# felixzhu17/Reranking-Multimodal-Retrievers

Hardware: AMD Instinct MI355X
Metric: reranked query x candidate pairs/sec at K=100, seq_len=512 (higher is better)
Workload: dtype fp16

## Files before the change

reranking-multimodal-retrievers_amd/build.py:

```python
from __future__ import annotations

import os
import subprocess
import sys
from concurrent.futures import ThreadPoolExecutor

HERE = os.path.dirname(os.path.abspath(__file__))
CSRC = os.path.join(HERE, "csrc")
LIB = os.path.join(HERE, "librerank_mi355.so")
SOURCES = ["rr_api.hip", "gemm_bf16.hip", "gemm_fp8.hip", "attention_bf16.hip", "elementwise.hip", "head.hip", "pair_assembly.hip", "li_scores.hip", "passage_bank.hip",
           "pair_tokenizer.cpp"]
HEADERS = [os.path.join(CSRC, "rr_common.h"), os.path.join(os.path.dirname(HERE), "include", "rerank_mi355.h"),
           os.path.join(os.path.dirname(HERE), "include", "rerank_mi355_diag.h"),
           os.path.join(CSRC, "unicode_tables.h")]
HIPCC = os.environ.get("HIPCC", "/opt/rocm/bin/hipcc")
FLAGS = ["--offload-arch=gfx950", "-O3", "-fPIC", "-std=c++17", "-Wall", "-Wno-unused-function", "-fno-slp-vectorize",
         *os.environ.get("RR_HIPCC_EXTRA", "").split()]
EXTRA = {"attention_bf16.hip": ["-fno-honor-nans", "-mno-amdgpu-ieee"]}


def _stale(target: str, deps) -> bool:
    if not os.path.exists(target):
        return True
    t = os.path.getmtime(target)
    return any(os.path.getmtime(d) > t for d in deps)


OBJDUMP = os.path.join(os.path.dirname(os.path.dirname(HIPCC)), "lib", "llvm", "bin", "llvm-objdump")
NO_PACKED_F32 = ["gemm_bf16.o", "gemm_fp8.o", "elementwise.o", "pair_assembly.o", "li_scores.o", "passage_bank.o"]


def check_no_packed_f32(obj: str) -> None:
    import re
    import shutil
    import tempfile
    if not os.path.exists(OBJDUMP):
        raise RuntimeError(f"{OBJDUMP} not found: cannot verify the packed-f32 rule for {obj}")
    d = tempfile.mkdtemp(prefix="rr_isa_")
    try:
        local = os.path.join(d, os.path.basename(obj))
        shutil.copy(obj, local)
        subprocess.run([OBJDUMP, "--offloading", local], cwd=d, capture_output=True, text=True, check=True)
        dev = [f for f in os.listdir(d) if "gfx950" in f]
        if len(dev) != 1:
            raise RuntimeError(f"no gfx950 code object in {obj}")
        dis = subprocess.run([OBJDUMP, "-d", os.path.join(d, dev[0])], capture_output=True, text=True, check=True).stdout
        bad = re.findall(r"v_pk_(?:add|mul)_f32[^\n]*", dis)
        ins = [l.split("//")[0].strip() for l in dis.splitlines() if l.startswith("\t")]
        for i, l in enumerate(ins):
            if i and l.startswith("v_pk_fma_f32") and ins[i - 1].startswith("s_waitcnt"):
                bad.append(l + "   (behind " + ins[i - 1] + ")")
        if bad:
            raise RuntimeError(f"{os.path.basename(obj)}: {len(bad)} packed-f32 instructions in the device code (first: {bad[0].strip()}); "
                               "build with -fno-slp-vectorize (reranking-multimodal-retrievers_amd/build.py FLAGS)")
    finally:
        shutil.rmtree(d, ignore_errors=True)


LAST_BUILD: dict = {}


def build_library(force: bool = False, verbose: bool = False) -> str:
    import json
    import time
    lib_existed = os.path.exists(LIB)
    objdir = os.path.join(HERE, "build")
    os.makedirs(objdir, exist_ok=True)
    jobs = []
    for s in SOURCES:
        src = os.path.join(CSRC, s)
        obj = os.path.join(objdir, os.path.splitext(s)[0] + ".o")
        if force or _stale(obj, [src] + HEADERS):
            if s.endswith(".cpp"):
                jobs.append([HIPCC, "-O2", "-fPIC", "-std=c++17", "-Wall", "-pthread", "-c", src, "-o", obj])
            else:
                jobs.append([HIPCC, *FLAGS, *EXTRA.get(s, []), "-c", src, "-o", obj])

    def run(cmd):
        if verbose:
            print(" ".join(cmd), flush=True)
        r = subprocess.run(cmd, capture_output=True, text=True)
        if r.returncode != 0:
            raise RuntimeError("hipcc failed:\n" + " ".join(cmd) + "\n" + r.stdout + r.stderr)
        return r.stderr

    with ThreadPoolExecutor(max_workers=4) as ex:
        list(ex.map(run, jobs))
    objs = [os.path.join(objdir, os.path.splitext(s)[0] + ".o") for s in SOURCES]
    if force or jobs or _stale(LIB, objs):
        for o in NO_PACKED_F32:
            obj = os.path.join(objdir, o)
            try:
                check_no_packed_f32(obj)
            except RuntimeError:
                os.remove(obj)
                raise
        run([HIPCC, "--offload-arch=gfx950", "-shared", "-fPIC", "-pthread", "-o", LIB, *objs])
        linked = True
    else:
        linked = False
    LAST_BUILD.clear()
    LAST_BUILD.update(compiled=[os.path.basename(j[-3]) for j in jobs], linked=linked, reused_prebuilt_library=lib_existed and not linked,
                      forced=bool(force), when=time.strftime("%Y-%m-%dT%H:%M:%S"))
    try:
        with open(os.path.join(objdir, "build_record.json"), "w") as f:
            json.dump(LAST_BUILD, f, indent=1)
    except OSError:
        pass
    return LIB


if __name__ == "__main__":
    print(build_library(force="--force" in sys.argv, verbose=True))
```

reranking-multimodal-retrievers_amd/csrc/gemm_bf16.hip:

```cpp
#include "rr_common.h"

#include <atomic>
#include <cstdlib>
#include <mutex>

#ifndef RR_EPI_DIAG
#define RR_EPI_DIAG 0
#endif

namespace {

constexpr int BK = 64;
__device__ __forceinline__ int k_walk_reversed(int n0) { return (n0 >> 10) & 1; }

__device__ __forceinline__ void lds_barrier() {
  asm volatile("s_waitcnt lgkmcnt(0)" ::: "memory");
  __builtin_amdgcn_s_barrier();
  asm volatile("" ::: "memory");
}

template <int N>
__device__ __forceinline__ void wait_vmcnt() {
  if constexpr (N == 0) asm volatile("s_waitcnt vmcnt(0)" ::: "memory");
  else if constexpr (N == 2) asm volatile("s_waitcnt vmcnt(2)" ::: "memory");
  else if constexpr (N == 4) asm volatile("s_waitcnt vmcnt(4)" ::: "memory");
  else if constexpr (N == 6) asm volatile("s_waitcnt vmcnt(6)" ::: "memory");
  else if constexpr (N == 8) asm volatile("s_waitcnt vmcnt(8)" ::: "memory");
  else if constexpr (N == 10) asm volatile("s_waitcnt vmcnt(10)" ::: "memory");
  else if constexpr (N == 12) asm volatile("s_waitcnt vmcnt(12)" ::: "memory");
  else if constexpr (N == 16) asm volatile("s_waitcnt vmcnt(16)" ::: "memory");
  else if constexpr (N == 24) asm volatile("s_waitcnt vmcnt(24)" ::: "memory");
  else static_assert(N < 0, "add the vmcnt literal");
}

template <int PIECES, int MAXT>
__device__ __forceinline__ void wait_tiles(int tiles_in_flight) {
  if constexpr (MAXT >= 2) { if (tiles_in_flight >= 2) { wait_vmcnt<2 * PIECES>(); return; } }
  if constexpr (MAXT >= 1) { if (tiles_in_flight >= 1) { wait_vmcnt<PIECES>(); return; } }
  wait_vmcnt<0>();
}

__device__ __forceinline__ float fast_erf(float x) {
  const float ax = fabsf(x);
  const float t = __builtin_amdgcn_rcpf(fmaf(0.3275911f, ax, 1.0f));
  float p = fmaf(1.061405429f, t, -1.453152027f);
  p = fmaf(p, t, 1.421413741f);
  p = fmaf(p, t, -0.284496736f);
  p = fmaf(p, t, 0.254829592f);
  const float e = __expf(-ax * ax);
  const float r = fmaf(-p * t, e, 1.0f);
  return copysignf(r, x);
}
__device__ __forceinline__ float tanh_fast(float x) { return 1.0f - 2.0f * __builtin_amdgcn_rcpf(__expf(2.0f * x) + 1.0f); }
__device__ __forceinline__ float qgelu_fast(float x) { return x * __builtin_amdgcn_rcpf(1.0f + __expf(-1.702f * x)); }
__device__ __forceinline__ float gelu_fast(float x) { return gelu_erf_fast(x); }

struct LnResid {
  const float2* stats;
  const float* gamma;
  const float* beta;
  bf16_t* x16;
  int ldx;
  float2* part;
  int nparts;
  const float2* in_stats;
  const float* csum;
  int flags;
  const bf16_t* r_hi;
  const bf16_t* r_lo;
  int ld16;
  bf16_t* lo_out;
};
__device__ __forceinline__ float dpp_f(float old, float v, int ctrl, int row_mask, bool bound) {
  return __builtin_bit_cast(float, ctrl == 0x111 ? __builtin_amdgcn_update_dpp(__builtin_bit_cast(int, old), __builtin_bit_cast(int, v), 0x111, 0xf, 0xf, true)
                                   : ctrl == 0x112 ? __builtin_amdgcn_update_dpp(__builtin_bit_cast(int, old), __builtin_bit_cast(int, v), 0x112, 0xf, 0xf, true)
                                   : ctrl == 0x114 ? __builtin_amdgcn_update_dpp(__builtin_bit_cast(int, old), __builtin_bit_cast(int, v), 0x114, 0xf, 0xf, true)
                                   : ctrl == 0x118 ? __builtin_amdgcn_update_dpp(__builtin_bit_cast(int, old), __builtin_bit_cast(int, v), 0x118, 0xf, 0xf, true)
                                                   : __builtin_amdgcn_update_dpp(__builtin_bit_cast(int, old), __builtin_bit_cast(int, v), 0x142, 0xa, 0xf, false));
}
__device__ __forceinline__ float group32_sum(float v) {
  v += dpp_f(0.f, v, 0x111, 0xf, true);
  v += dpp_f(0.f, v, 0x112, 0xf, true);
  v += dpp_f(0.f, v, 0x114, 0xf, true);
  v += dpp_f(0.f, v, 0x118, 0xf, true);
  v += dpp_f(0.f, v, 0x142, 0xa, false);
  const int vi = __builtin_bit_cast(int, v);
  const float lo = __builtin_bit_cast(float, __builtin_amdgcn_readlane(vi, 31));
  const float hi = __builtin_bit_cast(float, __builtin_amdgcn_readlane(vi, 63));
  return (threadIdx.x & 32) ? hi : lo;
}
// ... 537 lines not shown
            const int gm = row_base + r, gcol = n0 + c * (16 / ES);
            const bool ok = i < ROWS * CPR && gm < M && gcol < N;
            float4 x = ok ? *(const float4*)(resid + (size_t)gm * ldr + gcol) : make_float4(0.f, 0.f, 0.f, 0.f);
            if (ln.stats) {
              const int gm_s = __builtin_amdgcn_readfirstlane(min(gm, M - 1));
              const float2 st2 = ln.stats[gm_s];
              x = make_float4((x.x - st2.x) * st2.y * lg.x + lb.x, (x.y - st2.x) * st2.y * lg.y + lb.y,
                              (x.z - st2.x) * st2.y * lg.z + lb.z, (x.w - st2.x) * st2.y * lg.w + lb.w);
            }
            rv[u] = x;
          }
        }
        static_assert((ROWS * CPR) % (512 * UNR) == 0, "every thread runs every step (cross-lane sums below)");
#pragma unroll
        for (int u = 0; u < UNR; ++u) {
          const int i = i0 + u * 512, r = i / CPR, c = i - r * CPR;
          const int gm = row_base + r, gcol = n0 + c * (16 / ES);
          const bool ok = i < ROWS * CPR && gm < M && gcol < N;
          float4 f = make_float4(0.f, 0.f, 0.f, 0.f);
          if (ok) {
            uint4 v = *(const uint4*)(lds + r * PITCH + c * 16);
            if (EPI == EPI_BIAS_RESID_F32) {
              f = __builtin_bit_cast(float4, v);
              f.x += rv[u].x; f.y += rv[u].y; f.z += rv[u].z; f.w += rv[u].w;
              v = __builtin_bit_cast(uint4, f);
            }
            *(uint4*)((char*)Cv + ((size_t)gm * ldc + gcol) * ES) = v;
          }
          if (EPI == EPI_BIAS_RESID_F32) { if (ln.x16) fold_emit<DT>(ln, f, ok, gm, gcol, N); }
        }
      }
      if (pass + 1 < NPASS) lds_barrier();
    }
  } else {
#pragma unroll
    for (int q = 0; q < 4; ++q) {
      const int hA = q >> 1, hB = q & 1;
#pragma unroll
      for (int nt = 0; nt < 2; ++nt) {
        const int gn = n0 + hB * 128 + wc * 32 + nt * 16 + (lane >> 4) * 4;
        if (gn >= N) continue;
        const float4 bv = (bias && !bias_done) ? *(const float4*)(bias + gn) : make_float4(0.f, 0.f, 0.f, 0.f);
#pragma unroll
        for (int mt = 0; mt < 4; ++mt) {
          const int gm = m0 + hA * 128 + wr * 64 + mt * 16 + (lane & 15);
          if (gm >= M) continue;
          float v0 = acc[q][nt][mt][0] + bv.x, v1 = acc[q][nt][mt][1] + bv.y, v2 = acc[q][nt][mt][2] + bv.z,
                v3 = acc[q][nt][mt][3] + bv.w;
          if (EPI == EPI_BIAS_GELU_BF16) { v0 = gelu_fast(v0); v1 = gelu_fast(v1); v2 = gelu_fast(v2); v3 = gelu_fast(v3); }
          if (EPI == EPI_BIAS_TANH_BF16) { v0 = tanh_fast(v0); v1 = tanh_fast(v1); v2 = tanh_fast(v2); v3 = tanh_fast(v3); }
          if (EPI == EPI_BIAS_QGELU_BF16) { v0 = qgelu_fast(v0); v1 = qgelu_fast(v1); v2 = qgelu_fast(v2); v3 = qgelu_fast(v3); }
          if (EPI == EPI_BIAS_RESID_F32) {
            const float4 rv = ln_apply(*(const float4*)(resid + (size_t)gm * ldr + gn), ln, gm, gn);
            v0 += rv.x; v1 += rv.y; v2 += rv.z; v3 += rv.w;
          }
          if (F32_OUT) *(float4*)((float*)Cv + (size_t)gm * ldc + gn) = make_float4(v0, v1, v2, v3);
          else *(uint2*)((bf16_t*)Cv + (size_t)gm * ldc + gn) = make_uint2(pack2<DT>(v0, v1), pack2<DT>(v2, v3));
        }
      }
    }
  }
  stamp(stamps, 3);
}

template <int EPI, int DT, int SPLIT = 0, int DIAG = 0, bool FOLD = false>
__global__ __launch_bounds__(512) void gemm_kernel_hp(const bf16_t* __restrict__ A, int lda,
                                                     const bf16_t* __restrict__ W, int ldw,
                                                     const float* __restrict__ bias,
                                                     const float* __restrict__ resid, int ldr,
                                                     void* __restrict__ Cv, int ldc, int M, int N, int Kd,
                                                     int tiles_n, int nwg, unsigned long long* stamps, LnResid ln,
                                                     int stagger_unit) {
  const bool mrev = stagger_unit >= 1000;
  if (mrev) stagger_unit -= 1000;
  const int GROUP = stagger_unit >= 50 && stagger_unit <= 55 ? (2 << (stagger_unit - 50))
                    : (stagger_unit == 56 || Kd > 1024 || (tiles_n <= 4 && stagger_unit != 57)) ? 1 : 8;
  if (stagger_unit >= 100) {
    const int n = (int)(blockIdx.x & 7) * (stagger_unit - 100);
    for (int i = 0; i < n; ++i) __builtin_amdgcn_s_sleep(4);
  }
  stamp(stamps, 0);
  constexpr int BM = 256, BN = 256, HALF = 128 * 128;
  constexpr bool FOLD_IN = FOLD && EPI != EPI_BIAS_RESID_F32, FOLD_OUT = FOLD && EPI == EPI_BIAS_RESID_F32;
  extern __shared__ __attribute__((aligned(16))) char lds[];

  const int bid = blockIdx.x, gstep = (int)(gridDim.x >> 3);
  const int xcd = bid & 7, q8 = nwg >> 3, r8 = nwg & 7;
  const int chunk0 = xcd < r8 ? xcd * (q8 + 1) : r8 * (q8 + 1) + (xcd - r8) * q8, chunk_n = q8 + (xcd < r8 ? 1 : 0);
  int li = bid >> 3;
  if (li >= chunk_n) return;
  int m0, n0;
  const int tiles_m = nwg / tiles_n;
  const bool serp = stagger_unit != 59;
  int krev = 0;
  auto tile_origin = [&](int gidx, int& m0_, int& n0_) {
    const int per_group = GROUP * tiles_n, grp = gidx / per_group, r = gidx - grp * per_group;
    const int rows = min(GROUP, tiles_m - grp * GROUP);
    const int tn = r / rows, tm = grp * GROUP + (r - tn * rows);
    m0_ = tm * BM;
    n0_ = tn * BN;
    krev = serp ? k_walk_reversed(n0_) : 0;
  };
  tile_origin(chunk0 + (mrev ? chunk_n - 1 - li : li), m0, n0);

  const int tid = threadIdx.x, lane = tid & 63;
  const int wave = __builtin_amdgcn_readfirstlane(tid >> 6);
  const int wr = wave >> 2, wc = wave & 3;

  uint32_t so_a0[2], so_a1[2], so_b0[2], so_b1[2];
  const bf16_t *a_tile, *w_tile;
#define RR_SETUP_SRC(m0_, n0_)                                                                          \
  _Pragma("unroll") for (int i = 0; i < 2; ++i) {                                                       \
    const int r = (wave * 2 + i) * 8 + (lane >> 3);                       \
    const int c = (lane & 7) ^ ((r >> 1) & 7);                                                          \
    so_a0[i] = (uint32_t)(((size_t)min(r, M - 1 - (m0_)) * lda + c * 8) * 2);                           \
    so_a1[i] = (uint32_t)(((size_t)min(128 + r, M - 1 - (m0_)) * lda + c * 8) * 2);                     \
    so_b0[i] = (uint32_t)(((size_t)min(r, N - 1 - (n0_)) * ldw + c * 8) * 2);                           \
    so_b1[i] = (uint32_t)(((size_t)min(128 + r, N - 1 - (n0_)) * ldw + c * 8) * 2);                     \
  }                                                                                                     \
  a_tile = A + (size_t)(m0_) * lda;                                                                     \
  w_tile = W + (size_t)(n0_) * ldw;
  RR_SETUP_SRC(m0, n0)
  const uint32_t lds_base = lds_addr(lds);
  const int nk = Kd / BK, H = 4 * nk;
#define RR_DMA(t_, J)                                                                                             \
  {                                                                                                               \
    const uint32_t dst_ = __builtin_amdgcn_readfirstlane(lds_base + (((t_) & 1) * 4 + (J)) * HALF + wave * 2048); \
    const int tk_ = krev ? nk - 1 - (t_) : (t_);                      \
    const void* sb_ = ((J) == 0 || (J) == 3) ? (const void*)(a_tile + (size_t)tk_ * BK) : (const void*)(w_tile + (size_t)tk_ * BK); \
    const uint32_t* so_ = (J) == 0 ? so_a0 : (J) == 3 ? so_a1 : (J) == 1 ? so_b0 : so_b1;                         \
    glds16_so(sb_, so_[0], dst_);                                                                                 \
    glds16_so(sb_, so_[1], dst_ + 1024);                                                                          \
  }
  auto wait_half = [&](int h_need, int h_last) {
    if (h_need >= H) return;
    const int after = h_last - h_need;
    if (after >= 3) wait_vmcnt<6>();
    else if (after == 2) wait_vmcnt<4>();
    else if (after == 1) wait_vmcnt<2>();
    else wait_vmcnt<0>();
  };

  const int a_off = swz128(wr * 64 + (lane & 15), lane >> 4);
  const int b_off = swz128(wc * 32 + (lane & 15), lane >> 4);
  const int lds_dup = (DIAG == 3 && (stagger_unit == 62 || stagger_unit == 63)) ? stagger_unit - 61 : 0;
  auto dup_read = [&](const char* p_) {
    if constexpr (DIAG == 3) {
      for (int d_ = 0; d_ < lds_dup; ++d_) {
        f32x4 scratch_;
        asm volatile("ds_read_b128 %0, %1" : "=v"(scratch_) : "v"(lds_addr(p_)) : "memory");
      }
    }
  };
  auto read_a = [&](const char* slot, int ks, bf16x8 (&f)[4]) {
    const char* b = slot + (ks ? (a_off ^ 64) : a_off);
#pragma unroll
    for (int mt = 0; mt < 4; ++mt) { f[mt] = *(const bf16x8*)(b + mt * 2048); dup_read(b + mt * 2048); }
  };
  auto read_b = [&](const char* slot, int ks, bf16x8 (&f)[2]) {
    const char* b = slot + (ks ? (b_off ^ 64) : b_off);
#pragma unroll
    for (int nt = 0; nt < 2; ++nt) { f[nt] = *(const bf16x8*)(b + nt * 2048); dup_read(b + nt * 2048); }
  };

  f32x4 acc[4][2][4];

  bf16x8 AF0[4], AF1[4], B0K0[2], B0K1[2], B1K0[2], B1K1[2];

#define RR_BLK(Q, AF, BF)                                                                          \
  _Pragma("unroll") for (int nt = 0; nt < 2; ++nt) _Pragma("unroll") for (int mt = 0; mt < 4; ++mt)  \
      acc[Q][nt][mt] = mfma16<DT>(BF[nt], AF[mt], acc[Q][nt][mt]);
#define RR_SBAR() __builtin_amdgcn_sched_barrier(0)
#define RR_PRIO(p) __builtin_amdgcn_s_setprio(p);

  constexpr int PARAM_OFF = 152 * 1024;
  auto stage_params = [&](int m0_, int n0_) {
    int lane_ = lane;
    asm volatile("" : "+v"(lane_));
    const int lane = lane_;
    if constexpr (FOLD_IN) {
      const int d = wave * 64 + lane;
      glds4_so(ln.in_stats + m0_, (uint32_t)((min(d >> 1, M - 1 - m0_) * 2 + (d & 1)) * 4),
               __builtin_amdgcn_readfirstlane(lds_base + PARAM_OFF + wave * 256));
    }
    if (wave < 4) {
      if (bias) glds4_so(bias + n0_, (uint32_t)(min(wave * 64 + lane, N - 1 - n0_) * 4),
                         __builtin_amdgcn_readfirstlane(lds_base + PARAM_OFF + 2048 + wave * 256));
    } else if (FOLD_IN) {
      glds4_so(ln.csum + n0_, (uint32_t)(min((wave - 4) * 64 + lane, N - 1 - n0_) * 4),
               __builtin_amdgcn_readfirstlane(lds_base + PARAM_OFF + 3072 + (wave - 4) * 256));
    }
    if (EPI == EPI_BIAS_RESID_F32 && ln.stats) {
      const int d = wave * 64 + lane;
      glds4_so(ln.stats + m0_, (uint32_t)((min(d >> 1, M - 1 - m0_) * 2 + (d & 1)) * 4),
               __builtin_amdgcn_readfirstlane(lds_base + PARAM_OFF + 6144 + wave * 256));
      glds4_so((wave < 4 ? ln.gamma : ln.beta) + n0_, (uint32_t)(min((wave & 3) * 64 + lane, N - 1 - n0_) * 4),
               __builtin_amdgcn_readfirstlane(lds_base + PARAM_OFF + 4096 + (wave >> 2) * 1024 + (wave & 3) * 256));
    }
  };
  if (!bias) {
    if (tid < 256) *(float*)(lds + PARAM_OFF + 2048 + tid * 4) = 0.f;
// ... 64 lines not shown
    if (d1) RR_DMA(t + 1, 3)                                  \
    RR_SBAR();                                                                                             \
    RR_MARK(2)                                                                                             \
    RR_PRIO(2)                                                                                             \
    RR_BLK(0, AF1, B0K1)                                                                                   \
    RR_SBAR();                                                                                             \
                                                                            \
    RR_MARK(3)                                                                                             \
    read_b(sl + 2 * HALF, 1, B1K1);                                                                        \
    RR_SBAR();                                                                                             \
    RR_PRIO(1)                                                                                             \
    RR_BLK(1, AF0, B1K0)                                                                                   \
    RR_SBAR();                                                                                             \
    RR_MARK(4)                                                                                             \
    read_a(sl + 3 * HALF, 0, AF0);                                                                         \
    RR_SBAR();                                                                                             \
    RR_PRIO(0)                                                                                             \
    RR_BLK(1, AF1, B1K1)                                                                                   \
    RR_SYNC(STEADY, 4, 4 * (t + 1) + 1, min(H - 1, 4 * (t + 1) + 3), 5)       \
    RR_ACC(0, 8)                                                                                           \
                                                                            \
    RR_MARK(0)                                                                                             \
    read_a(sl + 3 * HALF, 1, AF1);                                                                         \
    if (d2) RR_DMA(t + 2, 0)                                                \
    RR_SBAR();                                                                                             \
    RR_PRIO(3)                                                                                             \
    RR_BLK(3, AF0, B1K0)                                                                                   \
    RR_SBAR();                                                                                             \
    if (d2) RR_DMA(t + 2, 1)                                                                               \
    RR_SBAR();                                                                                             \
    RR_PRIO(2)                                                                                             \
    RR_BLK(3, AF1, B1K1)                                                                                   \
    RR_SBAR();                                                                                             \
    RR_MARK(1)                                                                                             \
                                                                            \
    RR_PRIO(1)                                                                                             \
    RR_BLK(2, AF0, B0K0)                                                                                   \
    RR_SBAR();                                                                                             \
    if ((STEADY) || t + 1 < nk) {                                                                          \
      read_a(sn + 0 * HALF, 0, AF0);                                                                       \
      read_b(sn + 1 * HALF, 0, B0K0);                                                                      \
    }                                                                                                      \
    if (d2) RR_DMA(t + 2, 2)                                                     \
    RR_SBAR();                                                                                             \
    RR_PRIO(0)                                                                                             \
    RR_BLK(2, AF1, B0K1)                                                                                   \
    RR_SYNC(STEADY, 6, 4 * (t + 1) + 3, min(H - 1, 4 * (t + 2) + 2), 2)       \
      \
    asm volatile("" : "+v"(AF0[0]), "+v"(AF0[1]), "+v"(AF0[2]), "+v"(AF0[3]), "+v"(B0K0[0]), "+v"(B0K0[1])); \
    RR_ACC(8, 5)                                                                                           \
  }
  const bool no_dma = DIAG == 2 && stagger_unit == 61;
  int t = 0;
  for (; t < nk - 2; ++t) RR_TILE(1)
  for (; t < nk; ++t) RR_TILE(0)
#undef RR_TILE
  if constexpr (DIAG == 2) {
    if (stamps && lane == 0) {
      asm volatile("s_waitcnt lgkmcnt(0)" ::: "memory");
      unsigned long long* o = stamps + (size_t)gridDim.x * 8 + ((size_t)blockIdx.x * 8 + wave) * 16;
      for (int k = 0; k < 13; ++k) o[k] = dg[k];
    }
  }
#undef RR_SYNC
#undef RR_MARK
#undef RR_ACC
  wait_vmcnt<0>();
  if (nk == 1) __builtin_amdgcn_s_barrier();
  if (first_tile) stamp(stamps, 2);
  EP_ADD(0)
  if constexpr (DIAG != 0) {
    if (stamps && tid == 0 && ep[11] < 32)
      stamps[(size_t)gridDim.x * 264 + (size_t)blockIdx.x * 64 + 2 * ep[11]] = __builtin_amdgcn_s_memrealtime();
  }

  const int cm0 = m0, cn0 = n0;
  li += gstep;
  const bool has_next = li < chunk_n;
  if (has_next) {
    tile_origin(chunk0 + (mrev ? chunk_n - 1 - li : li), m0, n0);
    RR_SETUP_SRC(m0, n0)
    RR_DMA(0, 0) RR_DMA(0, 1) RR_DMA(0, 2) RR_DMA(0, 3)
    if (nk > 1) RR_DMA(1, 0)
  }
  EP_ADD(1)

  constexpr bool F32_OUT = (EPI == EPI_BIAS_F32 || EPI == EPI_BIAS_RESID_F32);
  {
    constexpr int ES = F32_OUT ? 4 : 2;
    constexpr int PITCH = BN * ES + 16;
    constexpr int CPR = BN * ES / 16;
    constexpr int NPASS = F32_OUT ? 4 : 2;
    constexpr int ROWS = F32_OUT ? 64 : 128;
    static_assert(ROWS * PITCH <= 5 * HALF, "staging image must fit above the five prefetch slots");
    char* const stg = lds + 5 * HALF;
    int tid_o_ = tid;
    asm volatile("" : "+v"(tid_o_));
    const int tid = tid_o_, lane = tid_o_ & 63;
    auto activate = [&](f32x4 ab) -> f32x4 {
      float v0 = ab[0], v1 = ab[1], v2 = ab[2], v3 = ab[3];
      if constexpr (EPI == EPI_BIAS_GELU_BF16 && RR_PK_GELU != 0) {
        const f32x2 g0 = gelu_erf_fast2(f32x2{v0, v1}), g1 = gelu_erf_fast2(f32x2{v2, v3});
        return f32x4{g0.x, g0.y, g1.x, g1.y};
      }
      if (EPI == EPI_BIAS_GELU_BF16) { v0 = gelu_fast(v0); v1 = gelu_fast(v1); v2 = gelu_fast(v2); v3 = gelu_fast(v3); }
      if (EPI == EPI_BIAS_TANH_BF16) { v0 = tanh_fast(v0); v1 = tanh_fast(v1); v2 = tanh_fast(v2); v3 = tanh_fast(v3); }
      if (EPI == EPI_BIAS_QGELU_BF16) { v0 = qgelu_fast(v0); v1 = qgelu_fast(v1); v2 = qgelu_fast(v2); v3 = qgelu_fast(v3); }
      return f32x4{v0, v1, v2, v3};
    };
    const char* const pcol = lds + PARAM_OFF + 2048 + (wc * 32 + (lane >> 4) * 4) * 4;
    if constexpr (FOLD_IN) {
      float2 fst[2][4];
#pragma unroll
      for (int hA = 0; hA < 2; ++hA)
#pragma unroll
        for (int mt = 0; mt < 4; ++mt)
          fst[hA][mt] = *(const float2*)(lds + PARAM_OFF + (hA * 128 + wr * 64 + mt * 16 + (lane & 15)) * 8);
      float4 bv_n = *(const float4*)(pcol), cs_n = *(const float4*)(pcol + 1024);
#pragma unroll
      for (int it = 0; it < 8; ++it) {
        const int q = it >> 1, nt = it & 1;
        const float4 bv = bv_n, cs = cs_n;
        if (it + 1 < 8) {
          const int o = ((((it + 1) >> 1) & 1) * 128 + ((it + 1) & 1) * 16) * 4;
          bv_n = *(const float4*)(pcol + o);
          cs_n = *(const float4*)(pcol + 1024 + o);
        }
        RR_SBAR();
#pragma unroll
        for (int mt = 0; mt < 4; ++mt) acc[q][nt][mt] = activate(fold_apply(acc[q][nt][mt], fst[q >> 1][mt], cs, bv));
        RR_SBAR();
      }
    } else {
      float4 bv_n = *(const float4*)(pcol);
#pragma unroll
      for (int it = 0; it < 8; ++it) {
        const int q = it >> 1, nt = it & 1;
        const float4 bv = bv_n;
        if (it + 1 < 8) bv_n = *(const float4*)(pcol + ((((it + 1) >> 1) & 1) * 128 + ((it + 1) & 1) * 16) * 4);
        RR_SBAR();
#pragma unroll
        for (int mt = 0; mt < 4; ++mt)
          acc[q][nt][mt] = activate(f32x4{acc[q][nt][mt][0] + bv.x, acc[q][nt][mt][1] + bv.y, acc[q][nt][mt][2] + bv.z, acc[q][nt][mt][3] + bv.w});
        RR_SBAR();
      }
    }
    EP_ADD(2)
    const int my_col = (EPI == EPI_BIAS_RESID_F32 && SPLIT != 0) ? cn0 + (tid & 31) * 8 : cn0 + (tid % CPR) * (16 / ES);
    auto load_gb = [&](float4& lg, float4& lb, float4& lg1, float4& lb1) {
      lg = make_float4(1.f, 1.f, 1.f, 1.f); lb = make_float4(0.f, 0.f, 0.f, 0.f); lg1 = lg; lb1 = lb;
      if (EPI == EPI_BIAS_RESID_F32 && ln.stats && my_col < N) {
        const char* pp = lds + PARAM_OFF + 4096 + (my_col - cn0) * 4;
        lg = *(const float4*)pp;
        lb = *(const float4*)(pp + 1024);
        if constexpr (SPLIT != 0) { lg1 = *(const float4*)(pp + 16); lb1 = *(const float4*)(pp + 1024 + 16); }
      }
    };
    auto touch_resid = [&](int pass_) {
      if (EPI != EPI_BIAS_RESID_F32 || !(ln.flags & 1)) return;
      if (cm0 + 256 > M || cn0 + 256 > N) return;
      const size_t row0 = (size_t)(cm0 + (pass_ >> 1) * 128 + (pass_ & 1) * 64);
      if constexpr ((SPLIT & 1) != 0) {
        if constexpr ((SPLIT & 8) != 0) {
          if (wave < 4) {
            const bf16_t* sb = ln.r_hi + row0 * ln.ld16 + cn0;
            const uint32_t vo = (uint32_t)((((tid & 255) >> 2) * ln.ld16 + (tid & 3) * 64) * 2);
            glds4_so(sb, vo, __builtin_amdgcn_readfirstlane(lds_base + 5 * HALF + ROWS * PITCH + wave * 256));
          } else if (wave < 6) {
            const uint8_t* sb = (const uint8_t*)ln.r_lo + (row0 >> 5) * 16 * (size_t)(2 * ln.ld16) + cn0 * 2;
            const uint32_t vo = (uint32_t)(((tid & 127) >> 2) * (2 * ln.ld16) + (tid & 3) * 128);
            glds4_so(sb, vo, __builtin_amdgcn_readfirstlane(lds_base + 5 * HALF + ROWS * PITCH + wave * 256));
          }
        } else {
        const bf16_t* sb = (wave < 4 ? ln.r_hi : ln.r_lo) + row0 * ln.ld16 + cn0;
        const uint32_t vo = (uint32_t)((((tid & 255) >> 2) * ln.ld16 + (tid & 3) * 64) * 2);
        glds4_so(sb, vo, __builtin_amdgcn_readfirstlane(lds_base + 5 * HALF + ROWS * PITCH + wave * 256));
        }
      } else {
        const float* sb = resid + row0 * ldr + cn0;
        const uint32_t vo = (uint32_t)(((tid >> 3) * ldr + (tid & 7) * 32) * 4);
        glds4_so(sb, vo, __builtin_amdgcn_readfirstlane(lds_base + 5 * HALF + ROWS * PITCH + wave * 256));
      }
    };
    static_assert(5 * HALF + ROWS * PITCH + (F32_OUT ? 8 * 256 : 0) <= PARAM_OFF, "staging image + touch area must end below the parameter block");
    touch_resid(0);
    constexpr int UN8 = 4;
    const int c8 = tid & 31, gcol8 = cn0 + c8 * 8;
    const bool col_ok8 = gcol8 < N;
    constexpr bool SPLIT_EPI = (EPI == EPI_BIAS_RESID_F32 && SPLIT != 0);
    constexpr bool LO8 = SPLIT_EPI && (SPLIT & 8) != 0;
    constexpr float LO8_MX = 1.0f / (float)(1 << RR_LO8_SHIFT);
    uint4 rh[SPLIT_EPI ? UN8 : 1], rl[(SPLIT_EPI && !LO8) ? UN8 : 1];
    uint4 rl8[LO8 ? UN8 / 2 : 1];
    float4 ra[(SPLIT_EPI && !(SPLIT & 1)) ? UN8 : 1], rb[(SPLIT_EPI && !(SPLIT & 1)) ? UN8 : 1];
    auto issue_resid = [&](int pass_) {
      if constexpr (SPLIT_EPI) {
        const int rbase_ = cm0 + (pass_ >> 1) * 128 + (pass_ & 1) * 64;
#pragma unroll
        for (int u = 0; u < UN8; ++u) {
          const int gm = rbase_ + (tid >> 5) + u * 16;
          const bool ok = gm < M && col_ok8;
          if constexpr ((SPLIT & 1) != 0 && (RR_EPI_DIAG & 2) != 0) {
            rh[u] = make_uint4(0x3c003c00u + gm, 0x3c003c00u, 0x3c003c00u, 0x3c003c00u);
            rl[u] = make_uint4(0x10001000u + tid, 0x10001000u, 0x10001000u, 0x10001000u);
          } else if constexpr ((SPLIT & 1) != 0 && LO8) {
            rh[u] = ok ? load_stream_u4(ln.r_hi + (size_t)gm * ln.ld16 + gcol8) : make_uint4(0u, 0u, 0u, 0u);
            if (!(u & 1)) rl8[u >> 1] = ok ? load_stream_u4((const uint8_t*)ln.r_lo + lo8_pair_offset(gm, gcol8, ln.ld16)) : make_uint4(0u, 0u, 0u, 0u);
          } else if constexpr ((SPLIT & 1) != 0) {
            rh[u] = ok ? load_stream_u4(ln.r_hi + (size_t)gm * ln.ld16 + gcol8) : make_uint4(0u, 0u, 0u, 0u);
            if constexpr ((RR_EPI_DIAG & 8) != 0) rl[u] = (ok && !(u & 1)) ? load_stream_u4(ln.r_lo + (size_t)gm * ln.ld16 + gcol8) : make_uint4(0u, 0u, 0u, 0u);
            else rl[u] = ok ? load_stream_u4(ln.r_lo + (size_t)gm * ln.ld16 + gcol8) : make_uint4(0u, 0u, 0u, 0u);
          } else {
            ra[u] = ok ? load_stream_f4(resid + (size_t)gm * ldr + gcol8) : make_float4(0.f, 0.f, 0.f, 0.f);
            rb[u] = ok ? load_stream_f4(resid + (size_t)gm * ldr + gcol8 + 4) : make_float4(0.f, 0.f, 0.f, 0.f);
          }
        }
      }
    };
    issue_resid(0);
    EP_ADD(6)
    for (int pass = 0; pass < NPASS; ++pass) {
#pragma unroll
      for (int q = 0; q < 4; ++q) {
        const int hA = q >> 1, hB = q & 1;
        if (F32_OUT ? (hA != (pass >> 1) || wr != (pass & 1)) : (hA != pass)) continue;
#pragma unroll
        for (int nt = 0; nt < 2; ++nt) {
          const int cn = hB * 128 + wc * 32 + nt * 16 + (lane >> 4) * 4;
#pragma unroll
          for (int mt = 0; mt < 4; ++mt) {
// ... 123 lines not shown
              store_stream(cp, make_float4(f[0], f[1], f[2], f[3]));
              store_stream(cp + 4, make_float4(f[4], f[5], f[6], f[7]));
            }
          }
          if constexpr (SPLIT != 4 && (RR_EPI_DIAG & 4) == 0) {
            const int grp = gcol >> 7;
            const float rcnt = __builtin_amdgcn_rcpf((float)max(1, min(128, N - (grp << 7))));
            const float mg = row16_sum(((f[0] + f[1]) + (f[2] + f[3])) + ((f[4] + f[5]) + (f[6] + f[7]))) * rcnt;
            float q = 0.f;
            if (ok) {
#pragma unroll
              for (int j = 0; j < 8; ++j) q += (f[j] - mg) * (f[j] - mg);
            }
            const float m2 = row16_sum(q);
            if (st_ok && (tid & 15) == 0 && ((RR_EPI_DIAG & 16) == 0 || mg == 1.2345e38f)) ln.part[(size_t)gm * ln.nparts + grp] = make_float2(mg, m2);
          }
        }
        EP_ADD(8)
        if (pass + 1 < NPASS) issue_resid(pass + 1);
        EP_ADD(6)
      } else {
      constexpr int UNR = 8;
      static_assert(512 % CPR == 0 && ROWS * CPR == 512 * UNR, "one batch per pass; a wave must not straddle rows");
      if constexpr (EPI != EPI_BIAS_RESID_F32) {
#pragma unroll
        for (int h = 0; h < 2; ++h) {
          uint4 sv[UNR / 2];
#pragma unroll
          for (int u = 0; u < UNR / 2; ++u) {
            const int i = tid + (h * (UNR / 2) + u) * 512, r = i / CPR, c = i - r * CPR;
            sv[u] = *(const uint4*)(stg + r * PITCH + c * 16);
          }
          const bool sw = !F32_OUT && (tid & 256);
#pragma unroll
          for (int u = 0; u < UNR / 2; ++u) {
            const int i = tid + (h * (UNR / 2) + u) * 512, r = i / CPR, c = i - r * CPR;
            const int gm = row_base + r, gcol = cn0 + c * (16 / ES);
            const uint4 v = make_uint4(sw ? sv[u].z : sv[u].x, sw ? sv[u].w : sv[u].y, sw ? sv[u].x : sv[u].z, sw ? sv[u].y : sv[u].w);
            if (gm < M && gcol < N) store_stream((char*)Cv + ((size_t)gm * ldc + gcol) * ES, v);
          }
          RR_SBAR();
        }
      } else {
      float4 lg, lb, lg1, lb1;
      load_gb(lg, lb, lg1, lb1);
#pragma unroll
      for (int h = 0; h < 2; ++h) {
        constexpr int UH = UNR / 2;
        float4 rv[UH];
#pragma unroll
        for (int u = 0; u < UH; ++u) {
          const int i = tid + (h * UH + u) * 512, r = i / CPR, c = i - r * CPR;
          const int gm = row_base + r, gcol = cn0 + c * (16 / ES);
          const bool ok = gm < M && gcol < N;
          float4 x = ok ? load_stream_f4(resid + (size_t)gm * ldr + gcol) : make_float4(0.f, 0.f, 0.f, 0.f);
          if (ln.stats) {
            const float2 st2 = *(const float2*)(lds + PARAM_OFF + 6144 + (gm - cm0) * 8);
            x = make_float4((x.x - st2.x) * st2.y * lg.x + lb.x, (x.y - st2.x) * st2.y * lg.y + lb.y,
                            (x.z - st2.x) * st2.y * lg.z + lb.z, (x.w - st2.x) * st2.y * lg.w + lb.w);
          }
          rv[u] = x;
        }
#pragma unroll
        for (int u = 0; u < UH; ++u) {
          const int i = tid + (h * UH + u) * 512, r = i / CPR, c = i - r * CPR;
          const int gm = row_base + r, gcol = cn0 + c * (16 / ES);
          const bool ok = gm < M && gcol < N;
          float4 f = make_float4(0.f, 0.f, 0.f, 0.f);
          if (ok) {
            f = *(const float4*)(stg + r * PITCH + c * 16);
            f.x += rv[u].x; f.y += rv[u].y; f.z += rv[u].z; f.w += rv[u].w;
            store_stream((char*)Cv + ((size_t)gm * ldc + gcol) * ES, f);
          }
          if constexpr (FOLD_OUT) { if (ln.x16) fold_emit<DT>(ln, f, ok, gm, gcol, N); }
        }
        RR_SBAR();
      }
      }
      }
      EP_ADD(8)
      lds_barrier();
      EP_ADD(9)
    }
  }
  if (first_tile) stamp(stamps, 3);
  first_tile = false;
  if constexpr (DIAG != 0) {
    if (stamps && tid == 0 && ep[11] < 32)
      stamps[(size_t)gridDim.x * 264 + (size_t)blockIdx.x * 64 + 2 * ep[11] + 1] = __builtin_amdgcn_s_memrealtime();
    ep[11] += 1;
  }
  if (!has_next) break;
  stage_params(m0, n0);
  if (nk > 1) { RR_DMA(1, 1) RR_DMA(1, 2) }
  EP_ADD(10)
  }
  if constexpr (DIAG != 0) {
    if (stamps && lane == 0) {
      unsigned long long* o = stamps + (size_t)gridDim.x * 8 + (size_t)gridDim.x * 128 + ((size_t)blockIdx.x * 8 + wave) * 16;
      for (int k = 0; k < 12; ++k) o[k] = ep[k];
    }
  }
#undef EP_MARK
#undef EP_ADD
#undef RR_SETUP_SRC
#undef RR_DMA
#undef RR_BLK
#undef RR_SBAR
}



unsigned long long* g_stamps = nullptr;
std::atomic<int> g_resid_touch{0};
std::atomic<int> g_variant{-1};

inline hipError_t ensure_lds_attr(const void* kern, int lds_bytes, std::atomic<unsigned long long>& mask) {
  int dev = 0;
  hipError_t e = hipGetDevice(&dev);
  if (e != hipSuccess) return e;
  if (dev >= 0 && dev < 64 && ((mask.load(std::memory_order_acquire) >> dev) & 1ull)) return hipSuccess;
  e = hipFuncSetAttribute(kern, hipFuncAttributeMaxDynamicSharedMemorySize, lds_bytes);
  if (e != hipSuccess) return e;
  if (dev >= 0 && dev < 64) mask.fetch_or(1ull << dev, std::memory_order_release);
  return hipSuccess;
}
inline int device_cus() {
  static std::atomic<int> cache[64];
  int dev = 0;
  if (hipGetDevice(&dev) != hipSuccess) return 0;
  if (dev >= 0 && dev < 64) { const int c = cache[dev].load(std::memory_order_relaxed); if (c) return c; }
  hipDeviceProp_t prop;
  if (hipGetDeviceProperties(&prop, dev) != hipSuccess) return 0;
  const int n = prop.multiProcessorCount & ~7;
  if (dev >= 0 && dev < 64) cache[dev].store(n, std::memory_order_relaxed);
  return n;
}
std::atomic<int> g_grid_cus{0};
inline int persistent_cus() {
  const int n = device_cus(), lim = g_grid_cus.load();
  return lim >= 8 && lim < n ? (lim & ~7) : n;
}

int g_stagger = 0;
std::atomic<int> g_resid_fast{1};
std::atomic<int> g_desync{0};
inline int desync_arg(int Kd, int epilogue, int nwg, int n_cu) {
  const int pct = g_desync.load();
  if (pct <= 0 || nwg < 8 * n_cu) return 0;
  const long main_cyc = (long)(Kd / 64) * 2700;
  const long epi_cyc = epilogue == EPI_BIAS_RESID_F32 ? 30000 : epilogue == EPI_BIAS_GELU_BF16 ? 16000 : 8000;
  const long u = (main_cyc + epi_cyc) * pct / 100 / 8 / 256;
  return u > 0 ? 100 + (int)(u > 1000 ? 1000 : u) : 0;
}
int g_persistent = 1;

template <int DT>
hipError_t launch_hp(const bf16_t* A, int lda, const bf16_t* W, int ldw, const float* bias, const float* resid,
                     int ldr, void* C, int ldc, int M, int N, int Kd, int epilogue, hipStream_t st, LnResid ln) {
  if (N & 7) return hipErrorInvalidValue;
  const int tiles_m = (M + 255) / 256, tiles_n = (N + 255) / 256, nwg = tiles_m * tiles_n;
  const int n_cu = persistent_cus();
  if (n_cu < 8) return hipErrorInvalidValue;
  constexpr int lds_bytes = 160 * 1024;
  dim3 grid(nwg < n_cu ? ((nwg + 7) & ~7) : n_cu), block(512);
  unsigned long long* stamps = g_stamps;
  const int desync = desync_arg(Kd, epilogue, nwg, n_cu);
  const int mrev = nwg >= 2 * n_cu ? rr_m_direction_next() : 0;
#define RR_GEMM_CASE_F(E, F)                                                                                  \
  {                                                                                                           \
    auto kern = gemm_kernel_hp<E, DT, 0, 0, F>;                                                               \
    static std::atomic<unsigned long long> attr_mask{0};      \
    {                                                                                                         \
      hipError_t e = ensure_lds_attr((const void*)kern, lds_bytes, attr_mask);                                \
      if (e != hipSuccess) return e;                                                                          \
    }                                                                                                         \
    hipLaunchKernelGGL(kern, grid, block, lds_bytes, st, A, lda, W, ldw, bias, resid, ldr, C, ldc, M, N, Kd,  \
// ... 320 lines not shown
```

Baseline: 9517.

## Add per-wave LDS-slice epilogue for 16-bit GEMM outputs and prefetch next tile earlier

```diff
diff --git a/reranking-multimodal-retrievers_amd/build.py b/reranking-multimodal-retrievers_amd/build.py
--- a/reranking-multimodal-retrievers_amd/build.py
+++ b/reranking-multimodal-retrievers_amd/build.py
@@ -57,6 +57,42 @@
         shutil.rmtree(d, ignore_errors=True)
 
 
+READELF = os.path.join(os.path.dirname(OBJDUMP), "llvm-readelf")
+
+
+def check_ring_epilogue_registers(obj: str) -> None:
+    import re
+    import shutil
+    import tempfile
+    if not os.path.exists(READELF):
+        raise RuntimeError(f"{READELF} not found: cannot verify the register use of {obj}")
+    d = tempfile.mkdtemp(prefix="rr_isa_")
+    try:
+        local = os.path.join(d, os.path.basename(obj))
+        shutil.copy(obj, local)
+        subprocess.run([OBJDUMP, "--offloading", local], cwd=d, capture_output=True, text=True, check=True)
+        dev = [f for f in os.listdir(d) if "gfx950" in f]
+        if len(dev) != 1:
+            raise RuntimeError(f"no gfx950 code object in {obj}")
+        notes = subprocess.run([READELF, "--notes", os.path.join(d, dev[0])], capture_output=True, text=True, check=True).stdout
+        seen, bad = 0, []
+        for entry in re.split(r"\n\s+- \.agpr_count", notes)[1:]:
+            m = re.search(r"\.name:\s+\S*gemm_kernel_hpILi([0135])ELi(\d)ELi(\d+)ELi(\d)ELb([01])E", entry)
+            if not m:
+                continue
+            seen += 1
+            spill = int(re.search(r"\.vgpr_spill_count:\s+(\d+)", entry).group(1))
+            scratch = int(re.search(r"\.private_segment_fixed_size:\s+(\d+)", entry).group(1))
+            if spill or scratch:
+                bad.append(f"gemm_kernel_hp<{', '.join(m.groups())}>: .vgpr_spill_count {spill}, {scratch} B of scratch")
+        if not seen:
+            raise RuntimeError(f"{os.path.basename(obj)}: no 16-bit gemm_kernel_hp instantiation found in the code object's notes")
+        if bad:
+            raise RuntimeError(f"{os.path.basename(obj)}: " + "; ".join(bad))
+    finally:
+        shutil.rmtree(d, ignore_errors=True)
+
+
 LAST_BUILD: dict = {}
 
 
@@ -95,6 +131,12 @@
             except RuntimeError:
                 os.remove(obj)
                 raise
+        ring = os.path.join(objdir, "gemm_bf16.o")
+        try:
+            check_ring_epilogue_registers(ring)
+        except RuntimeError:
+            os.remove(ring)
+            raise
         run([HIPCC, "--offload-arch=gfx950", "-shared", "-fPIC", "-pthread", "-o", LIB, *objs])
         linked = True
     else:
diff --git a/reranking-multimodal-retrievers_amd/csrc/gemm_bf16.hip b/reranking-multimodal-retrievers_amd/csrc/gemm_bf16.hip
--- a/reranking-multimodal-retrievers_amd/csrc/gemm_bf16.hip
+++ b/reranking-multimodal-retrievers_amd/csrc/gemm_bf16.hip
@@ -6,6 +6,10 @@
 
 #ifndef RR_EPI_DIAG
 #define RR_EPI_DIAG 0
+#endif
+
+#ifndef RR_WAVE_EPI
+#define RR_WAVE_EPI 1
 #endif
 
 namespace {
@@ -709,6 +713,7 @@
   stamp(stamps, 0);
   constexpr int BM = 256, BN = 256, HALF = 128 * 128;
   constexpr bool FOLD_IN = FOLD && EPI != EPI_BIAS_RESID_F32, FOLD_OUT = FOLD && EPI == EPI_BIAS_RESID_F32;
+  constexpr bool WAVE_EPI = RR_WAVE_EPI != 0 && EPI != EPI_BIAS_F32 && EPI != EPI_BIAS_RESID_F32;
   extern __shared__ __attribute__((aligned(16))) char lds[];
 
   const int bid = blockIdx.x, gstep = (int)(gridDim.x >> 3);
@@ -742,8 +747,9 @@
     const int c = (lane & 7) ^ ((r >> 1) & 7);                                                          \
     so_a0[i] = (uint32_t)(((size_t)min(r, M - 1 - (m0_)) * lda + c * 8) * 2);                           \
     so_a1[i] = (uint32_t)(((size_t)min(128 + r, M - 1 - (m0_)) * lda + c * 8) * 2);                     \
-    so_b0[i] = (uint32_t)(((size_t)min(r, N - 1 - (n0_)) * ldw + c * 8) * 2);                           \
-    so_b1[i] = (uint32_t)(((size_t)min(128 + r, N - 1 - (n0_)) * ldw + c * 8) * 2);                     \
+    const int rb = WAVE_EPI ? (r >> 5) * 64 + (r & 31) : r;   \
+    so_b0[i] = (uint32_t)(((size_t)min(rb, N - 1 - (n0_)) * ldw + c * 8) * 2);                          \
+    so_b1[i] = (uint32_t)(((size_t)min((WAVE_EPI ? 32 : 128) + rb, N - 1 - (n0_)) * ldw + c * 8) * 2);  \
   }                                                                                                     \
   a_tile = A + (size_t)(m0_) * lda;                                                                     \
   w_tile = W + (size_t)(n0_) * ldw;
@@ -974,6 +980,7 @@
     RR_SETUP_SRC(m0, n0)
     RR_DMA(0, 0) RR_DMA(0, 1) RR_DMA(0, 2) RR_DMA(0, 3)
     if (nk > 1) RR_DMA(1, 0)
+    if constexpr (WAVE_EPI) { if (nk > 1) { RR_DMA(1, 1) RR_DMA(1, 2) } }
   }
   EP_ADD(1)
 
@@ -1000,7 +1007,8 @@
       if (EPI == EPI_BIAS_QGELU_BF16) { v0 = qgelu_fast(v0); v1 = qgelu_fast(v1); v2 = qgelu_fast(v2); v3 = qgelu_fast(v3); }
       return f32x4{v0, v1, v2, v3};
     };
-    const char* const pcol = lds + PARAM_OFF + 2048 + (wc * 32 + (lane >> 4) * 4) * 4;
+    const char* const pcol = lds + PARAM_OFF + 2048 + (wc * (WAVE_EPI ? 64 : 32) + (lane >> 4) * 4) * 4;
+    auto pofs = [](int it) { return (((it >> 1) & 1) * (WAVE_EPI ? 32 : 128) + (it & 1) * 16) * 4; };
     if constexpr (FOLD_IN) {
       float2 fst[2][4];
 #pragma unroll
@@ -1014,7 +1022,7 @@
         const int q = it >> 1, nt = it & 1;
         const float4 bv = bv_n, cs = cs_n;
         if (it + 1 < 8) {
-          const int o = ((((it + 1) >> 1) & 1) * 128 + ((it + 1) & 1) * 16) * 4;
+          const int o = pofs(it + 1);
           bv_n = *(const float4*)(pcol + o);
           cs_n = *(const float4*)(pcol + 1024 + o);
         }
@@ -1029,7 +1037,7 @@
       for (int it = 0; it < 8; ++it) {
         const int q = it >> 1, nt = it & 1;
         const float4 bv = bv_n;
-        if (it + 1 < 8) bv_n = *(const float4*)(pcol + ((((it + 1) >> 1) & 1) * 128 + ((it + 1) & 1) * 16) * 4);
+        if (it + 1 < 8) bv_n = *(const float4*)(pcol + pofs(it + 1));
         RR_SBAR();
 #pragma unroll
         for (int mt = 0; mt < 4; ++mt)
@@ -1038,6 +1046,43 @@
       }
     }
     EP_ADD(2)
+    if constexpr (WAVE_EPI) {
+      const int r16 = lane & 15;
+      char* const slice = lds + 8 * HALF + wave * 2048;
+      const int wofs = r16 * 128 + ((((lane >> 5) ^ r16) & 7) * 16) + ((((lane >> 4) ^ (r16 >> 3)) & 1) * 8);
+      const int rofs = (lane >> 3) * 128 + (((lane & 7) ^ (lane >> 3)) * 16);
+      const int grow = cm0 + wr * 64 + (lane >> 3), gcol = cn0 + wc * 64 + (lane & 7) * 8;
+      const bool col_ok = gcol < N;
+      char* const cp = (char*)Cv + ((size_t)grow * ldc + gcol) * 2;
+      auto slab_write = [&](int s) {
+        const int hA = s >> 2, mt = s & 3;
+#pragma unroll
+        for (int hB = 0; hB < 2; ++hB)
+#pragma unroll
+          for (int nt = 0; nt < 2; ++nt) {
+            const f32x4 v = acc[hA * 2 + hB][nt][mt];
+            *(uint2*)(slice + (wofs ^ (hB * 64 + nt * 32))) = make_uint2(pack2<DT>(v[0], v[1]), pack2<DT>(v[2], v[3]));
+          }
+      };
+      RR_SBAR();
+      wait_vmcnt<0>();
+      RR_SBAR();
+      EP_ADD(4)
+      slab_write(0);
+#pragma unroll
+      for (int s = 0; s < 8; ++s) {
+        asm volatile("" ::: "memory");
+        const uint4 v0 = *(const uint4*)(slice + rofs), v1 = *(const uint4*)(slice + rofs + 1024);
+        asm volatile("" ::: "memory");
+        if (s + 1 < 8) slab_write(s + 1);
+        const int ro = (s >> 2) * 128 + (s & 3) * 16;
+        if (col_ok && grow + ro < M) store_stream(cp + (size_t)ro * ldc * 2, v0);
+        if (col_ok && grow + ro + 8 < M) store_stream(cp + (size_t)(ro + 8) * ldc * 2, make_uint4(v1.z, v1.w, v1.x, v1.y));
+      }
+      EP_ADD(8)
+      if (has_next) __builtin_amdgcn_s_barrier();
+      EP_ADD(9)
+    } else {
     const int my_col = (EPI == EPI_BIAS_RESID_F32 && SPLIT != 0) ? cn0 + (tid & 31) * 8 : cn0 + (tid % CPR) * (16 / ES);
     auto load_gb = [&](float4& lg, float4& lb, float4& lg1, float4& lb1) {
       lg = make_float4(1.f, 1.f, 1.f, 1.f); lb = make_float4(0.f, 0.f, 0.f, 0.f); lg1 = lg; lb1 = lb;
@@ -1327,6 +1372,7 @@
       lds_barrier();
       EP_ADD(9)
     }
+    }
   }
   if (first_tile) stamp(stamps, 3);
   first_tile = false;
@@ -1337,7 +1383,7 @@
   }
   if (!has_next) break;
   stage_params(m0, n0);
-  if (nk > 1) { RR_DMA(1, 1) RR_DMA(1, 2) }
+  if constexpr (!WAVE_EPI) { if (nk > 1) { RR_DMA(1, 1) RR_DMA(1, 2) } }
   EP_ADD(10)
   }
   if constexpr (DIAG != 0) {
```

Result: no change. 9602 (median of 6 runs) (+0.9%).
